# sfu-rsl/FastTrack

Hardware: AMD Instinct MI355X
Metric: frames/sec extract+match (higher is better)
Workload: dtype u8

## Files before the change

### fasttrack_amd/_capi.py

```python
from __future__ import annotations

import ctypes as C
import os
import re

import numpy as np

_PKG = os.path.dirname(os.path.abspath(__file__))
LIB_PATH = os.environ.get("FT_LIB") or os.path.join(_PKG, "libfasttrack_amd.so")
HEADER_PATH = os.path.join(os.path.dirname(_PKG), "include", "fasttrack_amd.h")

FT_OK, FT_ERR_INVALID, FT_ERR_NO_DEVICE, FT_ERR_HIP, FT_ERR_CAPACITY, FT_ERR_EMPTY = 0, -1, -2, -3, -4, -5

KP_DTYPE = np.dtype([("x", "<f4"), ("y", "<f4"), ("size", "<f4"), ("angle", "<f4"), ("response", "<f4"),
                     ("octave", "<i4"), ("class_id", "<i4")])
assert KP_DTYPE.itemsize == 28


class FastTrackError(RuntimeError):
    def __init__(self, status: int, message: str):
        super().__init__(f"fasttrack_amd status {status}: {message}")
        self.status = status


# ... 194 lines not shown
    L.ft_tracked_frame_search_keyframe_projection.argtypes = [vp, C.POINTER(KeyFramePoints), C.POINTER(SE3), f, f, i, i, vp, ip]
    L.ft_tracked_batch_create.argtypes = [vp, i, i, i, C.POINTER(vp)]
    L.ft_tracked_batch_destroy.argtypes = [vp]
    L.ft_tracked_batch_upload.argtypes = [vp, i, C.POINTER(FrameView)]
    L.ft_tracked_batch_search_last_frame.argtypes = [vp, i, C.POINTER(LastPoints), vp, f, vp, vp, i, C.POINTER(vp), vp]
    L.ft_tracked_batch_search_last_frame_se3.argtypes = [vp, i, C.POINTER(LastPoints), C.POINTER(SE3), C.POINTER(SE3), f, vp, vp, i,
                                                         C.POINTER(vp), vp]
    L.ft_tracked_batch_track_local_map.argtypes = [vp, i, C.POINTER(FramePose), C.POINTER(MapPoints), f, f, f, f, i, f,
                                                   C.POINTER(FrustumResult), vp, C.POINTER(vp), vp]
    L.ft_tracked_batch_submit_search_last_frame.argtypes = L.ft_tracked_batch_search_last_frame.argtypes
    L.ft_tracked_batch_submit_search_last_frame_se3.argtypes = L.ft_tracked_batch_search_last_frame_se3.argtypes
    L.ft_tracked_batch_submit_track_local_map.argtypes = L.ft_tracked_batch_track_local_map.argtypes
    L.ft_tracked_batch_wait.argtypes = [vp]
    L.ft_tracked_batch_holder_obs.argtypes = [vp, i, vp]
    L.ft_tracked_batch_bind_fisheye.argtypes = [vp, vp, vp, i, i, i, i, i, i, C.POINTER(FrameView), C.POINTER(FisheyeRig), vp, C.POINTER(vp),
                                                C.POINTER(vp), C.POINTER(vp), C.POINTER(vp), vp]
    L.ft_tracked_batch_bind_fisheye_slots.argtypes = [vp, vp, vp, i, i, i, i, i, i, i, C.POINTER(FrameView), C.POINTER(FisheyeRig), vp,
                                                      C.POINTER(vp), C.POINTER(vp), C.POINTER(vp), C.POINTER(vp), vp]
    L.ft_descriptor_distance.argtypes = [vp, vp, vp, i, vp]
    L.ft_stereo_frontend_device_descriptors.argtypes = [vp, i, i, C.POINTER(vp), ip]
    L.ft_vocabulary_create.argtypes = [vp, i, i, i, i, i, vp, vp, vp, vp, C.POINTER(vp)]
    L.ft_vocabulary_load_text.argtypes = [vp, C.c_char_p, C.POINTER(vp)]
    L.ft_vocabulary_destroy.argtypes = [vp]
    L.ft_vocabulary_info.argtypes = [vp, ip, ip, ip, ip]
    L.ft_bow_transform.argtypes = [vp, vp, i, i, i, vp, vp, vp, vp, vp, i, ip, vp, vp, vp, i, ip]
    L.ft_search_by_bow.argtypes = [vp, C.POINTER(BowSide), vp, C.POINTER(BowSide), i, f, i, vp, ip]
    L.ft_search_for_triangulation.argtypes = [vp, C.POINTER(TriangKeyFrame), i, C.POINTER(TriangKeyFrame), C.POINTER(TriangPair), i, i, i, vp, vp, vp]
    L.ft_fuse_search.argtypes = [vp, C.POINTER(FusePoints), i, C.POINTER(FuseTarget), vp, vp, vp, vp]
    L.ft_search_keyframe_sim3.argtypes = [vp, C.POINTER(FrameView), i, C.POINTER(Sim3Job)]
    L.ft_selftest_libm.argtypes = [vp, i, C.c_uint32, C.c_uint32, C.c_uint32, C.POINTER(C.c_ulonglong),
                                   C.POINTER(C.c_ulonglong), C.POINTER(C.c_uint32)]
    L.ft_octree_distribute.argtypes = [vp, i, i, i, i, i, i, vp, i, ip]
    L.ft_level_geometry.argtypes = [i, i, i, f, i, vp, vp, vp, vp, vp, vp, vp]
    _lib = L
    return L


def check(status: int) -> None:
    if status != FT_OK:
        raise FastTrackError(status, lib().ft_last_error().decode(errors="replace"))


def ptr(a):
    return None if a is None else a.ctypes.data_as(C.c_void_p)
```

### fasttrack_amd/csrc/extractor.cpp

```cpp
#include <algorithm>
#include <map>
#include <cmath>
#include <cstdio>
#include <cstdlib>
#include <cstring>

#include "ft_host.h"

namespace {

inline int cvRoundF(float v) { return (int)lrintf(v); }
inline short satShort(int v) { return (short)(v < -32768 ? -32768 : (v > 32767 ? 32767 : v)); }

#define FT_REQUIRE(cond, msg)                      \
    do {                                           \
        if (!(cond)) {                             \
            ft_set_error(std::string(msg));        \
            return FT_ERR_INVALID;                 \
        }                                          \
    } while (0)

void buildTaps(int ssize, int dsize, bool clampIndex, FtTap *out) {
    const double inv_scale = (double)dsize / ssize;
    const double scale = 1. / inv_scale;
// ... 72 lines not shown
        v.cellBase = cellBase;
        v.cellCap = ((v.wCell + 1) / 2) * ((v.hCell + 1) / 2);
        FT_REQUIRE(v.cellCap < 65536 && v.wCell + 6 < 256 && v.hCell + 6 < 256, "FAST cell too large for the cell records");
        g.fastLv[l] = (unsigned)v.pitch | ((unsigned)v.cellCap << 16);
        v.stageBase = stageBase;
        v.candBase = candBase;
        v.candCap = nCols * nRows * v.cellCap;
        cellBase += nCols * nRows;
        stageBase += v.candCap;
        candBase += v.candCap;
        if (l >= 1) {
            const FtLevelGeom &p = g.lv[l - 1];
            v.area2x = (p.w == 2 * v.w && p.h == 2 * v.h) ? 1 : 0;
            v.xtab = tapOff;
            tapOff += v.w;
            v.ytab = tapOff;
            tapOff += v.h;
        }
        ex->levelMax[l] = ft::octree_max_result(minB, v.maxBX, minB, v.maxBY, ex->quota[l]);
        maxKp += ex->levelMax[l];
    }
    g.totalCells = cellBase;
    g.stagePerSlot = stageBase;
    g.candPerSlot = candBase;
    g.pyrPerSlot = pyrOff;
    g.maxKp = maxKp;
    taps.assign(std::max(tapOff, 1), FtTap{0, 0, 0, 0});
    for (int l = 1; l < L; l++) {
        buildTaps(g.lv[l - 1].w, g.lv[l].w, true, &taps[g.lv[l].xtab]);
        buildTaps(g.lv[l - 1].h, g.lv[l].h, false, &taps[g.lv[l].ytab]);
    }
    return FT_OK;
}

template <typename T>
int devAlloc(T **p, size_t n) {
    FT_HIP(hipMalloc((void **)p, std::max<size_t>(n, 1) * sizeof(T)));
    return FT_OK;
}
template <typename T>
int pinAlloc(T **p, size_t n, unsigned flags = hipHostMallocDefault) {
    FT_HIP(hipHostMalloc((void **)p, std::max<size_t>(n, 1) * sizeof(T), flags));
    return FT_OK;
}

void freeAll(ft_extractor *ex) {
    hipSetDevice(ex->ctx->device);
    if (ex->stream) hipStreamSynchronize(ex->stream);
    if (ex->streamB) hipStreamSynchronize(ex->streamB);
    for (int i = 0; i < FT_OCT_STREAMS; i++)
        if (ex->streamO[i]) hipStreamSynchronize(ex->streamO[i]);
    if (ex->octLayout.prof) {
        unsigned long long h[FT_MAX_LEVELS * 8];
        if (hipMemcpy(h, ex->octLayout.prof, sizeof h, hipMemcpyDeviceToHost) == hipSuccess)
            for (int l = 0; l < ex->nlevels; l++)
                fprintf(stderr, "[oct profile] level %d: codes %.1f us  sort %.1f us  rounds %.1f us (std::sort replay %.1f us, %llu elems in %llu sorts)  pick %.1f us\n",
                        l, h[l * 8] * 0.01, h[l * 8 + 1] * 0.01, h[l * 8 + 2] * 0.01, h[l * 8 + 4] * 0.01, h[l * 8 + 5], h[l * 8 + 6], h[l * 8 + 3] * 0.01);
        hipFree(ex->octLayout.prof);
        ex->octLayout.prof = nullptr;
    }
    ex->evt.destroy();
    for (int i = 0; i < FT_PIPE_MAX; i++) {
        if (ex->evA[i]) hipEventDestroy(ex->evA[i]);
        if (ex->evB[i]) hipEventDestroy(ex->evB[i]);
        if (ex->evO[i]) hipEventDestroy(ex->evO[i]);
    }
// ... 170 lines not shown
            ex->h_srcTab[b].ptr = images[b];
            ex->h_srcTab[b].stride = stride;
            continue;
        }
        uint8_t *stg = ex->h_stage + (size_t)b * width * height;
        for (int y = 0; y < height; y++) memcpy(stg + (size_t)y * width, images[b] + (size_t)y * stride, width);
        ex->h_srcTab[b].ptr = stg;
        ex->h_srcTab[b].stride = width;
    }
}

int ft_extract_ensure_host_cand(ft_extractor *ex) {
    if (ex->h_cand) return FT_OK;
    const size_t n = std::max<size_t>((size_t)ex->maxBatch * ex->geom.candPerSlot, 1);
    FT_HIP(hipHostMalloc((void **)&ex->h_cand, n * sizeof(uint32_t), hipHostMallocMapped | hipHostMallocCoherent));
    void *dp = nullptr;
    FT_HIP(hipHostGetDevicePointer(&dp, ex->h_cand, 0));
    ex->d_cand = (uint32_t *)dp;
    return FT_OK;
}

int ft_extract_launch_a(ft_extractor *ex, int b0, int nb, hipEvent_t done) {
    const FtGeom &g = ex->geom;
    if (!ex->deviceOctree) {
        const int rce = ft_extract_ensure_host_cand(ex);
        if (rce != FT_OK) return rce;
    }
    const bool tm = ex->ctx->kernelTiming;
    const int al = ex->l0Aligned ? 1 : 0;
    const uint8_t *const *l0 = ex->d_l0 + b0;
    uint8_t *pyr = ex->d_pyr + (size_t)b0 * g.pyrPerSlot;
    int *cellCount = ex->d_cellCount + (size_t)b0 * g.totalCells;
    uint32_t *stage = ex->d_stage + (size_t)b0 * g.stagePerSlot;
    ex->evt.begin(tm, "kernel.pyr_down(all levels)", ex->stream);
    int rc = ft_launch_pyramid(ex->stream, g, nb, l0, ex->l0pitch, pyr, ex->d_taps, al, ex->tune.pyr_rows);
    ex->evt.end(tm, ex->stream);
    if (rc != FT_OK) return rc;
    ex->evt.begin(tm, "kernel.fast_cells", ex->stream);
    rc = ft_launch_fast_cells(ex->stream, g, nb, l0, ex->l0pitch, pyr, ex->iniTh, ex->minTh, al, cellCount, stage,
                              ex->deviceOctree ? 0 : 1, ex->d_cellTab);
    ex->evt.end(tm, ex->stream);
    if (rc != FT_OK) return rc;
    ex->evt.begin(tm, "kernel.compact", ex->stream);
    uint32_t *candDst = ex->deviceOctree ? ex->d_candDev : ex->d_cand;
    int *cntDst = ex->deviceOctree ? ex->d_candCountDev : ex->d_candCount;
    rc = ft_launch_compact(ex->stream, g, nb, cellCount, stage, candDst + (size_t)b0 * g.candPerSlot,
                           cntDst + (size_t)b0 * g.nlevels);
    ex->evt.end(tm, ex->stream);
    if (rc != FT_OK) return rc;
    if (done) FT_HIP(hipEventRecord(done, ex->stream));
    return FT_OK;
}

int ft_extract_launch_octree(ft_extractor *ex, int sub, int b0, int nb, hipEvent_t done) {
    const FtGeom &g = ex->geom;
    hipStream_t so = ex->streamO[sub % FT_OCT_STREAMS];
    FT_HIP(hipEventRecord(ex->evO[sub], ex->stream));
    FT_HIP(hipStreamWaitEvent(so, ex->evO[sub], 0));
    FtOctArgs a = ex->octLayout;
    a.cand = ex->d_candDev + (size_t)b0 * g.candPerSlot;
    a.candCount = ex->d_candCountDev + (size_t)b0 * g.nlevels;
    a.sel = ex->d_sel + (size_t)b0 * g.maxKp;
    a.selCount = ex->d_selCount + (size_t)b0 * g.nlevels;
    a.overflow = ex->d_overflow;
    a.ovSlot = ex->d_ovSlot + b0;
    a.low = ex->d_octLow ? ex->d_octLow + (size_t)b0 * g.nlevels * FT_OCT_MAXN : nullptr;
    const bool large = nb > 16 || ex->lastBatch > 16;
    const bool histNow = ex->histEnabled && (large ? ex->histGrid > 0 : ex->histOn);
// ... 273 lines not shown
int ft_extractor_create(ft_context *ctx, int nfeatures, float scale_factor, int nlevels, int ini_th_fast,
                        int min_th_fast, int image_width, int image_height, int max_batch, ft_extractor **out) {
    FT_REQUIRE(ctx && out, "ft_extractor_create: null argument");
    *out = nullptr;
    FT_REQUIRE(nfeatures > 0, "nfeatures must be positive");
    FT_REQUIRE(nlevels >= 1 && nlevels <= FT_MAX_LEVELS, "nlevels outside [1, 12]");
    FT_REQUIRE(scale_factor > 1.0f, "scaleFactor must exceed 1");
    FT_REQUIRE(min_th_fast >= 1 && ini_th_fast >= min_th_fast && ini_th_fast < 255,
               "FAST thresholds must satisfy 1 <= minThFAST <= iniThFAST < 255");
    FT_REQUIRE(image_width >= 2 * FT_EDGE_THRESHOLD + 8 && image_height >= 2 * FT_EDGE_THRESHOLD + 8,
               "image smaller than the 19-px border allows");
    FT_REQUIRE(max_batch >= 1 && max_batch <= 4096, "max_batch outside [1, 4096]");
    int rc = ft_set_device(ctx);
    if (rc != FT_OK) return rc;
    ft_extractor *ex = new ft_extractor();
    ex->ctx = ctx;
    ex->nfeatures = nfeatures;
    ex->scaleFactor = scale_factor;
    ex->nlevels = nlevels;
    ex->iniTh = ini_th_fast;
    ex->minTh = min_th_fast;
    ex->width = image_width;
    ex->height = image_height;
    ex->maxBatch = max_batch;
    ex->tune = ctx->tuning;
    std::vector<FtTap> taps;
    rc = buildGeometry(ex, taps);
    if (rc != FT_OK) {
        delete ex;
        return rc;
    }
    const FtGeom &g = ex->geom;
    const size_t B = max_batch;
#define FT_TRY(x)            \
    do {                     \
        rc = (x);            \
        if (rc != FT_OK) {   \
            freeAll(ex);     \
            delete ex;       \
            return rc;       \
        }                    \
    } while (0)
    {
        hipStream_t lanes[FT_LANE_STREAMS];
        FT_TRY(ft_context_take_lanes(ctx, max_batch <= 16, image_width, image_height, lanes, &ex->ownStreams));
        ex->stream = lanes[0];
        ex->streamB = lanes[1];
        for (int i = 0; i < FT_OCT_STREAMS; i++) ex->streamO[i] = lanes[2 + i];
    }
    hipError_t se = hipSuccess;
    for (int i = 0; i < FT_PIPE_MAX && se == hipSuccess; i++) {
        se = hipEventCreateWithFlags(&ex->evA[i], hipEventDisableTiming);
        if (se == hipSuccess) se = hipEventCreateWithFlags(&ex->evB[i], hipEventDisableTiming);
        if (se == hipSuccess) se = hipEventCreateWithFlags(&ex->evO[i], hipEventDisableTiming);
        if (se == hipSuccess && i == 0) se = hipEventCreateWithFlags(&ex->evJoin, hipEventDisableTiming);
        if (se == hipSuccess && i == 0) se = hipEventCreateWithFlags(&ex->evUp, hipEventDisableTiming);
    }
    if (se != hipSuccess) {
        freeAll(ex);
        delete ex;
        return ft_hip_fail(se, "stream / event creation", __FILE__, __LINE__);
    }
    FT_TRY(devAlloc(&ex->d_pyr, B * g.pyrPerSlot));
    FT_TRY(devAlloc(&ex->d_taps, taps.size()));
    FT_TRY(devAlloc(&ex->d_cellTab, (size_t)std::max(g.totalCells, 1)));
    FT_TRY(devAlloc(&ex->d_cellCount, B * g.totalCells));
// ... 148 lines not shown
        return FT_ERR_CAPACITY;
    }
    *n_out = k;
    if (k > capacity) {
        ft_set_error("ft_octree_distribute: capacity too small");
        return FT_ERR_CAPACITY;
    }
    for (int i = 0; i < k; i++) out_idx[i] = keep[i];
    return FT_OK;
}

int ft_level_geometry(int width, int height, int nfeatures, float scale_factor, int nlevels, int *level_w,
                      int *level_h, int *quota, int *n_cols, int *n_rows, int *w_cell, int *h_cell) {
    FT_REQUIRE(nlevels >= 1 && nlevels <= FT_MAX_LEVELS && scale_factor > 1.0f && nfeatures > 0, "bad parameters");
    ft_extractor ex;
    ex.nfeatures = nfeatures;
    ex.scaleFactor = scale_factor;
    ex.nlevels = nlevels;
    ex.width = width;
    ex.height = height;
    std::vector<FtTap> taps;
    int rc = buildGeometry(&ex, taps);
    if (rc != FT_OK) return rc;
    for (int l = 0; l < nlevels; l++) {
        const FtLevelGeom &v = ex.geom.lv[l];
        if (level_w) level_w[l] = v.w;
        if (level_h) level_h[l] = v.h;
        if (quota) quota[l] = ex.quota[l];
        if (n_cols) n_cols[l] = v.nCols;
        if (n_rows) n_rows[l] = v.nRows;
        if (w_cell) w_cell[l] = v.wCell;
        if (h_cell) h_cell[l] = v.hCell;
    }
    return FT_OK;
}

int ft_extractor_destroy(ft_extractor *ex) {
    if (!ex) return FT_OK;
    freeAll(ex);
    ex->ctx->liveObjects--;
    delete ex;
    return FT_OK;
}

int ft_extractor_levels(const ft_extractor *ex) { return ex ? ex->nlevels : 0; }
int ft_extractor_max_batch(const ft_extractor *ex) { return ex ? ex->maxBatch : 0; }
int ft_extractor_max_keypoints(const ft_extractor *ex) { return ex ? ex->geom.maxKp : 0; }

int ft_extractor_scale_factors(const ft_extractor *ex, float *scale, float *inv_scale, float *sigma2,
                               float *inv_sigma2) {
    FT_REQUIRE(ex, "null extractor");
    for (int i = 0; i < ex->nlevels; i++) {
        if (scale) scale[i] = ex->sf[i];
        if (inv_scale) inv_scale[i] = ex->invsf[i];
        if (sigma2) sigma2[i] = ex->sigma2[i];
        if (inv_sigma2) inv_sigma2[i] = ex->invsigma2[i];
    }
    return FT_OK;
}

int ft_extractor_features_per_level(const ft_extractor *ex, int *quota) {
    FT_REQUIRE(ex && quota, "null argument");
    for (int i = 0; i < ex->nlevels; i++) quota[i] = ex->quota[i];
    return FT_OK;
}

// ... 411 lines not shown
```

### fasttrack_amd/csrc/ft_host.h

```cpp
#pragma once

#include <atomic>
#include <chrono>
#include <map>
#include <mutex>
#include <string>
#include <vector>

#include "ft_internal.h"
#include "octree.h"
#include "thread_pool.h"

#define FT_PIPE_MAX 8
#define FT_LANE_SMALL_PIXELS ((size_t)600 * 1000)
#define FT_LANE_MAP_SMALL {1, 2, 3, 4, 2, 1, 3, 1, 5, 4, 3, 2, 1, 1, 0, 1}
#define FT_OCT_STREAMS 2
#define FT_LANE_STREAMS (2 + FT_OCT_STREAMS)

#define FT_TUNING_OPTIONS(X)                                                                                                  \
    X(pipeline_depth, "FT_PIPELINE_DEPTH", 0, 0, 8, "sub-batches a throughput batch is enqueued as (0 = automatic, 1 = no pipelining, <= 8)") \
    X(device_octree, "FT_DEVICE_OCTREE", 1, 0, 1, "DistributeOctTree on the device (0 = host thread pool)")                  \
    X(oct_hist, "FT_OCT_HIST", 1, 0, 1, "histogram tier of the device octree for levels above 4096 candidates")              \
    X(oct_hist_first, "FT_OCT_HIST_FIRST", 1, 0, 2, "histogram formulation for every level: 0 never, 1 latency-mode launches, 2 always") \
    X(oct_big, "FT_OCT_BIG", 1, 0, 1, "sorted big tier of the device octree (up to 16384 keys per level)")                   \
    X(pyr_rows, "FT_PYR_ROWS", 1, 0, 1, "pyramid of launches of 8+ images: 1 = row-streaming kernel (k_pyr_rows), 0 = tile kernel (k_pyr_down)") \
    X(upload_kernel, "FT_UPLOAD_KERNEL", 1, 0, 1, "latency mode: frames go up through k_upload instead of DMA copies")       \
    X(graph, "FT_GRAPH", 1, 0, 1, "latency mode: batches of <= 8 frames are captured and replayed as HIP graphs")            \
    X(paired, "FT_PAIRED", 1, 0, 1, "latency-mode stereo front ends run both cameras through one set of launches")           \
    X(pass_burst, "FT_PASS_BURST", 12, 2, 14, "projection searches: claim passes enqueued per host round trip")              \
    X(search_cache, "FT_SEARCH_CACHE", 2, 0, 3, "projection searches: 1 = later claim passes walk the cached candidate keys, 2 = and a batch of 24+ frames resolves its claims in one launch, 3 = every batch does") \
    X(search_grid, "FT_SEARCH_GRID", 1, 0, 1, "projection searches: CSR grid of the frame built on the device") \
    X(blocking_sync, "FT_BLOCKING_SYNC", 2, 0, 2, "host waits for the device: 0 = the runtime's default (it spins), 1 = sleeping (hipDeviceScheduleBlockingSync), 2 = sleeping when the process may use fewer than 8 CPUs")

struct ft_tuning {
#define FT_X(field, env, def, lo, hi, doc) int field = def;
    FT_TUNING_OPTIONS(FT_X)
#undef FT_X
};
bool ft_tuning_from_env(ft_tuning &t, std::string &err);
int *ft_tuning_field(ft_tuning &t, const char *name);
const char *ft_debug_env(const char *name);
const char *ft_read_env(const char *name);

struct ft_context {
    int device = 0;
    std::string deviceName;
    ft::ThreadPool *pool = nullptr;
    hipStream_t stream = nullptr;
    std::mutex laneMutex;
    std::vector<hipStream_t> lanes;
    hipStream_t uploadStream = nullptr;
    std::vector<int> laneMap;
    std::vector<int> laneMapSmall;
    bool userLaneMap = false;
    int nextLaneSet = 0;
    size_t maxPitch = 0;
    int hwQueues = 4;
    std::atomic<int> liveObjects{0};
// ... 44 lines not shown
        hipEventRecord(recs.back().b, st);
    }
    void resolve(ft_context *ctx) {
        for (auto &r : recs) {
            float ms = 0;
            if (hipEventElapsedTime(&ms, r.a, r.b) == hipSuccess) ctx->addStat(r.name, ms);
        }
        recs.clear();
        used = 0;
    }
    void destroy() {
        for (auto e : pool) hipEventDestroy(e);
        pool.clear();
    }
};

struct FtTimer {
    std::chrono::steady_clock::time_point t0 = std::chrono::steady_clock::now();
    double ms() const {
        return std::chrono::duration<double, std::milli>(std::chrono::steady_clock::now() - t0).count();
    }
};

struct ft_extractor {
    ft_context *ctx = nullptr;
    ft_tuning tune;
    int nfeatures = 0, nlevels = 0, iniTh = 0, minTh = 0, width = 0, height = 0, maxBatch = 0;
    float scaleFactor = 1.2f;
    std::vector<float> sf, invsf, sigma2, invsigma2;
    std::vector<int> quota;
    std::vector<int> levelMax;
    std::vector<int> levelOff;
    FtGeom geom{};
    hipStream_t stream = nullptr;
    hipStream_t streamB = nullptr;
    hipEvent_t evA[FT_PIPE_MAX] = {}, evB[FT_PIPE_MAX] = {};
    hipStream_t streamO[FT_OCT_STREAMS] = {};
    bool ownStreams = false;
    hipEvent_t evO[FT_PIPE_MAX] = {};
    struct GraphKey {
        int batch = 0, onDevice = 0, width = 0, height = 0, stride = 0, aligned = 0, bigGrid = 0;
        bool operator==(const GraphKey &o) const {
            return batch == o.batch && onDevice == o.onDevice && width == o.width && height == o.height && stride == o.stride &&
                   aligned == o.aligned && bigGrid == o.bigGrid;
        }
    } graphKey;
    hipGraphExec_t graphExec = nullptr;
    bool graphDisabled = false;
    hipEvent_t evJoin = nullptr;
    hipEvent_t evUp = nullptr;
    hipEvent_t foreignReader = nullptr;
    uint8_t *d_pyr = nullptr;
    FtTap *d_taps = nullptr;
    FtCellRec *d_cellTab = nullptr;
    int *d_cellCount = nullptr;
    uint32_t *d_stage = nullptr;
    const uint8_t **d_l0 = nullptr;
    const uint8_t **h_l0 = nullptr;
    uint8_t *h_stage = nullptr;
    FtSrcEntry *h_srcTab = nullptr;
    bool stageHost = false;
    float *d_sf = nullptr;
    uint32_t *h_cand = nullptr, *d_cand = nullptr;
    int *h_candCount = nullptr, *d_candCount = nullptr;
    bool deviceOctree = false;
    uint32_t *d_candDev = nullptr;
// ... 109 lines not shown
```

### fasttrack_amd/csrc/ft_internal.h

```cpp
#pragma once

#include <hip/hip_runtime.h>
#include <stdint.h>

#include <string>

#include "../../include/fasttrack_amd.h"

#define FT_MAX_LEVELS 12
#define FT_EDGE_THRESHOLD 19
#define FT_PATCH_SIZE 31
#define FT_HALF_PATCH 15
#define FT_TH_HIGH 100
#define FT_TH_LOW 50
#define FT_HISTO_LENGTH 30
#define FT_GRID_COLS 64
#define FT_GRID_ROWS 48

struct FtLevelGeom {
    int w, h, pitch;
    int off;
    int maxBX, maxBY;
    int nCols, nRows, wCell, hCell;
    int cellBase;
// ... 94 lines not shown
};

struct FtBowTree {
    const int *childStart;
    const unsigned *childList;
    const uint8_t *desc;
    const unsigned *wordId;
    const double *weight;
    int nNodes;
};
int ft_launch_bow_walk(hipStream_t st, const FtBowTree &t, const uint8_t *desc, int n, int nidLevel, unsigned *wordOut,
                       unsigned *nodeOut, double *weightOut);
struct FtBowSide {
    int n, nNodes;
    const unsigned *nodes;
    const int *offsets;
    const unsigned *features;
    const uint8_t *desc;
};
int ft_launch_search_by_bow(hipStream_t st, const FtBowSide &K, const uint8_t *kfHasPoint, const FtBowSide &F, int nleft,
                            float nnRatio, int *matches);

void ft_set_error(const std::string &msg);
int ft_debug_repeat(const char *name);
int ft_hip_fail(hipError_t e, const char *what, const char *file, int line);
const char *ft_debug_env(const char *name);

#define FT_HIP(call)                                                              \
    do {                                                                          \
        hipError_t _e = (call);                                                   \
        if (_e != hipSuccess) return ft_hip_fail(_e, #call, __FILE__, __LINE__);  \
    } while (0)

int ft_launch_pyramid(hipStream_t st, const FtGeom &g, int batch, const uint8_t *const *l0, int l0pitch,
                      uint8_t *pyr, const FtTap *taps, int alignedLoads, int rowsKernel);
struct FtCellRanges {
    int lo0, n0, lo1, n1;
};
int ft_launch_fast_cells(hipStream_t st, const FtGeom &g, int batch, const uint8_t *const *l0, int l0pitch,
                         const uint8_t *pyr, int iniTh, int minTh, int alignedLoads, int *cellCount,
                         uint32_t *stage, int ordered, const FtCellRec *cellTab);
int ft_launch_compact(hipStream_t st, const FtGeom &g, int batch, const int *cellCount, const uint32_t *stage,
                      uint32_t *cand, int *candCount);
int ft_launch_orient_desc(hipStream_t st, const FtGeom &g, int batch, const uint8_t *const *l0, int l0pitch,
                          const uint8_t *pyr, int alignedLoads, const FtSelKp *sel, const int *selCount,
                          const FtOctArgs &layout, int *nSel, ft_keypoint *keys, uint8_t *desc);
int ft_launch_octree(hipStream_t st, const FtGeom &g, int batch, const FtOctArgs &a);
int ft_launch_blur_level(hipStream_t st, const uint8_t *img, int pitch, int w, int h, uint8_t *dst, int dstPitch);
size_t ft_octree_smem_bytes(int poolCap, bool compact = false);
size_t ft_octree_hist_smem_bytes(int poolCap);
int ft_octree_big_keys(int poolCap);
size_t ft_fast_smem_bytes(const FtGeom &g);

struct __attribute__((aligned(16))) FtSortedR {
    float x, y;
    int octave, idx;
    unsigned long long desc[4];
};
struct FtStereoArgs {
    const ft_keypoint *keysL, *keysR;
    const uint8_t *descL, *descR;
    const int *nL, *nR;
    int capacity;
    float mbf, mb;
    float *uright, *depth;
    int *sad;
    int *hamIdx;
    int *nMatches;
// ... 62 lines not shown
```

### fasttrack_amd/csrc/kernels_extract.hip

```cpp
#include "ft_internal.h"
#include "libm_f32.h"
#include "wave_ops.h"

namespace {


struct FtMomentTab {
    unsigned W[17 * 8], M[17 * 8];
};
constexpr FtMomentTab ft_make_moment_tab() {
    constexpr int umax[16] = {15, 15, 15, 15, 14, 14, 14, 13, 13, 12, 11, 10, 9, 8, 6, 3};
    FtMomentTab t{};
    for (int av = 0; av < 16; av++)
        for (int j = 0; j < 8; j++)
            for (int k = 0; k < 4; k++) {
                const int u = -15 + 4 * j + k;
                const int au = u < 0 ? -u : u;
                if (u <= 15 && au <= umax[av]) {
                    t.W[av * 8 + j] |= (unsigned)(u + 16) << (8 * k);
                    t.M[av * 8 + j] |= 1u << (8 * k);
                }
            }
    return t;
}
// ... 153 lines not shown
    for (int j = 0; j < 4; j++) {
        const int dy = by + j;
        if (dy > dy1) break;
        const int sy0 = min(max((int)yt[j].s, 0), sh - 1) - sya, sy1 = min(max((int)yt[j].s + 1, 0), sh - 1) - sya;
        const uint8_t *r0 = T + __mul24(sy0, ldsPitch), *r1 = T + __mul24(sy1, ldsPitch);
        unsigned pk = 0;
#pragma unroll
        for (int k = 0; k < 4; k++) {
            const int h0 = r0[cx0[k]] * xt[k].a0 + r0[cx1[k]] * xt[k].a1;
            const int h1 = r1[cx0[k]] * xt[k].a0 + r1[cx1[k]] * xt[k].a1;
            pk |= (unsigned)(((vmul24((int)yt[j].a0, h0 >> 4) >> 16) + (vmul24((int)yt[j].a1, h1 >> 4) >> 16) + 2) >> 2) << (8 * k);
        }
        gstore<unsigned>(outLevel + (unsigned)vmad24(dy, D.pitch, bx), pk);
    }
}

#define PR_COLS 128
#ifndef PR_RB
#define PR_RB 32
#endif
#ifndef PR_PF
#define PR_PF 4
#endif
typedef unsigned short ft_us2 __attribute__((ext_vector_type(2)));
typedef unsigned ft_u2 __attribute__((ext_vector_type(2)));
__device__ __forceinline__ unsigned udot2_u16(unsigned a, unsigned b) {
    return __builtin_amdgcn_udot2(__builtin_bit_cast(ft_us2, a), __builtin_bit_cast(ft_us2, b), 0u, false);
}
__device__ __forceinline__ unsigned umulhi_su(unsigned bShifted16, unsigned a) {
    unsigned r;
    asm("v_mul_hi_u32 %0, %1, %2" : "=v"(r) : "s"(bShifted16), "v"(a));
    return r;
}
template <bool AREA>
__global__ __launch_bounds__(64) void k_pyr_rows(FtGeom g, int level, const uint8_t *const *l0, int l0pitch, uint8_t *pyr,
                                                 const FtTap *taps, FtSlotGrid sg, int stripsX, unsigned sxMagic,
                                                 int readableEnd) {
    const int lane = threadIdx.x;
    int slot, tile;
    if (!ft_slot_block(sg, slot, tile)) return;
    const int ty = div_by(tile, sxMagic), tx = tile - ty * stripsX;
    const FtLevelGeom &D = g.lv[level];
    int spitch;
    const uint8_t *S = level_ptr(g, level - 1, slot, l0, l0pitch, pyr, spitch);
    const int sw = g.lv[level - 1].w, sh = g.lv[level - 1].h;
    const int dx = tx * PR_COLS + 2 * lane;
    const int j0 = ty * PR_RB, nrows = min(PR_RB, D.h - j0);
    unsigned rowW0 = 0, rowW1 = 0;
    if constexpr (!AREA) {
        const ft_u2 t = gload<ft_u2>(taps + D.ytab + j0 + min(lane, nrows - 1));
        const int sy = (int)(short)(t.x & 0xffffu);
        rowW0 = (unsigned)min(max(sy, 0), sh - 1) | ((unsigned)min(max(sy + 1, 0), sh - 1) << 16);
        rowW1 = (t.x >> 16) | (t.y << 16);
        if (lane >= nrows) rowW0 = 0xffffffffu;
    }
    const int dxa = min(dx, D.w - 1), dxb = min(dx + 1, D.w - 1);
    int sxa, sxb, cxa, cxb;
    unsigned wa, wb;
    if constexpr (AREA) {
        sxa = 2 * dxa; sxb = 2 * dxb; cxa = sxa + 1; cxb = sxb + 1;
        wa = wb = 0x00010001u;
    } else {
        const ft_u2 ta = gload<ft_u2>(taps + D.xtab + dxa), tb = gload<ft_u2>(taps + D.xtab + dxb);
        sxa = (int)(short)(ta.x & 0xffffu); sxb = (int)(short)(tb.x & 0xffffu);
        cxa = min(sxa + 1, sw - 1); cxb = min(sxb + 1, sw - 1);
        wa = (ta.x >> 16) | (ta.y << 16);
        wb = (tb.x >> 16) | (tb.y << 16);
    }
    const int base = min(sxa & ~3, readableEnd - 8);
    const unsigned selA = (unsigned)(sxa - base) | 0x0c00u | ((unsigned)(cxa - base) << 16) | 0x0c000000u;
    const unsigned selB = (unsigned)(sxb - base) | 0x0c00u | ((unsigned)(cxb - base) << 16) | 0x0c000000u;
    auto rowTap = [&](int r, int &sy0, int &sy1, unsigned &b0, unsigned &b1) {
        if constexpr (AREA) {
            sy0 = 2 * (j0 + r); sy1 = r < nrows ? sy0 + 1 : -1; b0 = b1 = 0;
        } else {
            const unsigned w0 = (unsigned)__builtin_amdgcn_readlane((int)rowW0, r), w1 = (unsigned)__builtin_amdgcn_readlane((int)rowW1, r);
            sy0 = (int)(w0 & 0xffffu); sy1 = (int)(w0 >> 16);
            b0 = w1 << 16; b1 = w1 & 0xffff0000u;
        }
    };
// ... 37 lines not shown
                    asm volatile("" : "+v"(hpA), "+v"(hpB));
                }
                unsigned oA, oB;
                if constexpr (AREA) {
                    oA = (hpA + hcA + 2u) >> 2; oB = (hpB + hcB + 2u) >> 2;
                } else {
                    oA = (umulhi_su(b0, hpA) + umulhi_su(b1, hcA) + 2u) >> 2;
                    oB = (umulhi_su(b0, hpB) + umulhi_su(b1, hcB) + 2u) >> 2;
                }
                unsigned offD = laneDst + dOff;
                asm volatile("" : "+v"(offD));
                if constexpr (!EDGE) {
                    gstore<unsigned short>(dstBase + offD, (unsigned short)(oA | (oB << 8)));
                } else {
                    if (store2) gstore<unsigned short>(dstBase + offD, (unsigned short)(oA | (oB << 8)));
                    else if (store1) gstore<uint8_t>(dstBase + offD, (uint8_t)oA);
                }
                dOff += (unsigned)D.pitch;
                jr++;
                rowTap(jr, sy0, sy1, b0, b1);
            }
            r++;
        };
        for (int left = rLast - r + 1; left > 0; left -= PR_PF) {
#pragma unroll
            for (int k = 0; k < PR_PF; k++) {
                take(q[k]);
                step();
            }
        }
    };
    if (tx * PR_COLS + PR_COLS <= D.w) run(std::false_type{});
    else run(std::true_type{});
}

typedef unsigned short fs_us2 __attribute__((ext_vector_type(2)));
__device__ __forceinline__ unsigned pk_max_u16(unsigned a, unsigned b) {
    return __builtin_bit_cast(unsigned, __builtin_elementwise_max(__builtin_bit_cast(fs_us2, a), __builtin_bit_cast(fs_us2, b)));
}
__device__ __forceinline__ unsigned pk_min_u16(unsigned a, unsigned b) {
    return __builtin_bit_cast(unsigned, __builtin_elementwise_min(__builtin_bit_cast(fs_us2, a), __builtin_bit_cast(fs_us2, b)));
}
__device__ __forceinline__ bool has_arc9(unsigned m) {
    unsigned d = m | (m << 16);
    unsigned a = d & (d >> 1);
    a &= a >> 2;
    a &= a >> 4;
    a &= d >> 8;
    return (a & 0xffffu) != 0;
}

#define FT_RING(F)                                                                                            \
    F(0, 0, 3) F(1, 1, 3) F(2, 2, 2) F(3, 3, 1) F(4, 3, 0) F(5, 3, -1) F(6, 2, -2) F(7, 1, -3) F(8, 0, -3)    \
    F(9, -1, -3) F(10, -2, -2) F(11, -3, -1) F(12, -3, 0) F(13, -3, 1) F(14, -2, 2) F(15, -1, 3)

__device__ __forceinline__ int fast_score(int v, const int p[16]) {
    int mn3[16], mx3[16];
#pragma unroll
    for (int k = 0; k < 16; k++) {
        mn3[k] = min(min(p[k], p[(k + 1) & 15]), p[(k + 2) & 15]);
        mx3[k] = max(max(p[k], p[(k + 1) & 15]), p[(k + 2) & 15]);
    }
    int mn9[16], mx9[16];
#pragma unroll
    for (int k = 0; k < 16; k++) {
        mn9[k] = min(min(mn3[k], mn3[(k + 3) & 15]), mn3[(k + 6) & 15]);
// ... 964 lines not shown
        }
    }
    if (profW && lane == 0) atomicAdd(&g_odProf[0], 1ull);
}

}

static int fast_tile_pitch(const FtGeom &g) {
    int need = 0;
    for (int l = 0; l < g.nlevels; l++)
        if (g.lv[l].nCols * g.lv[l].nRows > 0) need = std::max(need, g.lv[l].wCell + 9);
    return need <= 48 ? 48 : (need <= 64 ? 64 : 0);
}

size_t ft_fast_smem_bytes(const FtGeom &g) {
    const int TP = fast_tile_pitch(g);
    size_t mxTile = 0, mxScore = 0, mxSum = 0;
    for (int l = 0; l < g.nlevels; l++) {
        const FtLevelGeom &L = g.lv[l];
        const size_t t = (size_t)fc_tile_bytes(L.wCell, L.hCell, TP), sc = (size_t)fc_score_bytes(L.wCell, L.hCell, TP);
        mxTile = std::max(mxTile, t);
        mxScore = std::max(mxScore, sc);
        mxSum = std::max(mxSum, t + sc);
    }
    return (TP ? mxTile + mxScore : mxSum) + fc_list_bytes();
}

static bool pyr_rows_fits(const FtGeom &g, int level) {
    const FtLevelGeom &D = g.lv[level], &P = g.lv[level - 1];
    return (double)P.w / (double)D.w < 2.5 && P.w >= 8;
}

int ft_launch_pyramid(hipStream_t st, const FtGeom &g, int batch, const uint8_t *const *l0, int l0pitch,
                      uint8_t *pyr, const FtTap *taps, int alignedLoads, int rowsKernel) {
    const bool rowsOn = rowsKernel != 0;
    for (int rep = ft_debug_repeat("pyr"); rep > 0; rep--)
    for (int level = 1; level < g.nlevels; level++) {
        const FtLevelGeom &D = g.lv[level], &P = g.lv[level - 1];
        if (rowsOn && batch >= 8 && alignedLoads && pyr_rows_fits(g, level)) {
            const int stripsX = (D.w + PR_COLS - 1) / PR_COLS, stripsY = (D.h + PR_RB - 1) / PR_RB;
            dim3 grid, block(64, 1, 1);
            const FtSlotGrid sg = ft_slot_grid(stripsX * stripsY, batch, grid);
            const int readableEnd = level == 1 ? std::min((P.w + 3) & ~3, l0pitch) : P.pitch;
            if (D.area2x)
                hipLaunchKernelGGL(k_pyr_rows<true>, grid, block, 0, st, g, level, l0, l0pitch, pyr, taps, sg, stripsX,
                                   div_magic_of((unsigned)stripsX), readableEnd);
            else
                hipLaunchKernelGGL(k_pyr_rows<false>, grid, block, 0, st, g, level, l0, l0pitch, pyr, taps, sg, stripsX,
                                   div_magic_of((unsigned)stripsX), readableEnd);
            continue;
        }
        const int cols = (int)((long long)PD_TW * P.w / D.w) + 8, rowsN = (int)((long long)PD_TH * P.h / D.h) + 8;
        const int ldsPitch = (cols + 3 + 3) & ~3;
        const unsigned sxQ16 = (unsigned)(((unsigned long long)P.w << 16) / (unsigned)D.w) + 1u;
        const unsigned syQ16 = (unsigned)(((unsigned long long)P.h << 16) / (unsigned)D.h) + 1u;
        const int tilesX = (D.w + PD_TW - 1) / PD_TW, tilesY = (D.h + PD_TH - 1) / PD_TH;
        dim3 grid, block(64, 1, 1);
        const FtSlotGrid sg = ft_slot_grid(tilesX * tilesY, batch, grid);
        hipLaunchKernelGGL(k_pyr_down, grid, block, (size_t)ldsPitch * rowsN + 4, st, g, level, l0, l0pitch, pyr, taps,
                           alignedLoads, ldsPitch, rowsN, sxQ16, syQ16, sg, tilesX, div_magic_of((unsigned)tilesX));
    }
    FT_HIP(hipGetLastError());
    return FT_OK;
}

static size_t fast_smem_of(const FtGeom &g, unsigned mask, int TP, int *tileBytes, int *scoreBytes) {
    size_t mxTile = 0, mxScore = 0, mxSum = 0;
    for (int l = 0; l < g.nlevels; l++) {
// ... 155 lines not shown
```

### include/fasttrack_amd.h

```cpp
#ifndef FASTTRACK_AMD_H
#define FASTTRACK_AMD_H

#include <stddef.h>
#include <stdint.h>

#ifdef __cplusplus
extern "C" {
#endif

#define FT_API __attribute__((visibility("default")))

typedef enum ft_status {
    FT_OK = 0,
    FT_ERR_INVALID = -1,
    FT_ERR_NO_DEVICE = -2,
    FT_ERR_HIP = -3,
    FT_ERR_CAPACITY = -4,
    FT_ERR_EMPTY = -5
} ft_status;

typedef struct ft_keypoint {
    float x, y, size, angle, response;
    int octave, class_id;
} ft_keypoint;
// ... 32 lines not shown
                               int min_th_fast, int image_width, int image_height, int max_batch,
                               ft_extractor **out);
FT_API int ft_extractor_destroy(ft_extractor *ex);
FT_API int ft_extractor_levels(const ft_extractor *ex);
FT_API int ft_extractor_max_batch(const ft_extractor *ex);
FT_API int ft_extractor_max_keypoints(const ft_extractor *ex);
FT_API int ft_extractor_scale_factors(const ft_extractor *ex, float *scale, float *inv_scale, float *sigma2,
                                      float *inv_sigma2);
FT_API int ft_extractor_features_per_level(const ft_extractor *ex, int *quota);
FT_API int ft_extractor_level_size(const ft_extractor *ex, int level, int *width, int *height);

FT_API int ft_extract(ft_extractor *ex, const uint8_t *image, int width, int height, int stride, int lap0,
                      int lap1, ft_keypoint *keypoints, uint8_t *descriptors, int capacity, int *n_keypoints,
                      int *n_mono);


FT_API int ft_extract_batch(ft_extractor *ex, const uint8_t *const *images, int batch, int on_device, int width,
                            int height, int stride, int lap0, int lap1, ft_keypoint *keypoints,
                            uint8_t *descriptors, int capacity, int *n_keypoints, int *n_mono);

FT_API int ft_extractor_download_level(ft_extractor *ex, int slot, int level, uint8_t *dst, int dst_stride);
FT_API int ft_extractor_download_blurred_level(ft_extractor *ex, int slot, int level, uint8_t *dst, int dst_stride);
FT_API int ft_extractor_device_level(ft_extractor *ex, int slot, int level, const uint8_t **dptr, int *pitch);
FT_API int ft_extractor_download_candidates(ft_extractor *ex, int slot, int level, int *xys, int capacity,
                                            int *n);

FT_API int ft_extractor_octree_on_device(ft_extractor *ex, int level, const int *xys, int n, int tiers, int *out_xys,
                                         int capacity, int *n_out, int *tier);

FT_API int ft_octree_distribute(const int *xys, int n, int minX, int maxX, int minY, int maxY, int N, int *out_idx,
                                int capacity, int *n_out);
FT_API int ft_level_geometry(int width, int height, int nfeatures, float scale_factor, int nlevels, int *level_w,
                             int *level_h, int *quota, int *n_cols, int *n_rows, int *w_cell, int *h_cell);

FT_API int ft_stereo_match(ft_extractor *exL, ft_extractor *exR, int slot, const ft_keypoint *keysL, int nL,
                           const ft_keypoint *keysR, int nR, const uint8_t *descL, const uint8_t *descR,
                           float mbf, float mb, int apply_median_cut, float *uright, float *depth, int *sad,
                           int *n_matches);

typedef struct ft_stereo_frontend ft_stereo_frontend;
FT_API int ft_stereo_frontend_create(ft_context *ctx, int nfeatures, float scale_factor, int nlevels,
                                     int ini_th_fast, int min_th_fast, int image_width, int image_height,
                                     int max_batch, float mbf, float mb, ft_stereo_frontend **out);
FT_API int ft_stereo_frontend_destroy(ft_stereo_frontend *fe);
FT_API ft_extractor *ft_stereo_frontend_left(ft_stereo_frontend *fe);
FT_API ft_extractor *ft_stereo_frontend_right(ft_stereo_frontend *fe);
FT_API int ft_stereo_frontend_submit(ft_stereo_frontend *fe, const uint8_t *const *imagesL,
                                     const uint8_t *const *imagesR, int batch, int on_device, int width, int height,
                                     int stride, ft_keypoint *keysL, uint8_t *descL, int *nL, ft_keypoint *keysR,
                                     uint8_t *descR, int *nR, int capacity, float *uright, float *depth,
                                     int *n_matches);
FT_API int ft_stereo_frontend_wait(ft_stereo_frontend *fe);
FT_API int ft_stereo_frontend_process(ft_stereo_frontend *fe, const uint8_t *const *imagesL,
                                      const uint8_t *const *imagesR, int batch, int on_device, int width,
                                      int height, int stride, ft_keypoint *keysL, uint8_t *descL, int *nL,
                                      ft_keypoint *keysR, uint8_t *descR, int *nR, int capacity, float *uright,
                                      float *depth, int *n_matches);
FT_API int ft_stereo_frontend_device_descriptors(ft_stereo_frontend *fe, int slot, int right, const uint8_t **dptr, int *n);

FT_API int ft_fisheye_match(ft_context *ctx, const uint8_t *descL, int nL, const uint8_t *descR, int nR,
                            int *matches, int *best, int *second);

typedef struct ft_fisheye_rig {
    float cam1[8], cam2[8];
    float precision;
    float Rlr[9], tlr[3];
// ... 283 lines not shown
```

Baseline: 79730.

## Fuse all pyramid levels into one cascade launch with per-band workgroups

Adds k_pyr_cascade, which builds every pyramid level in a single launch. Each workgroup of 16 waves owns a horizontal band of one image, with band row ranges precomputed on the host and widened so each band holds all source rows the next level needs. Workgroup barriers separate the levels, so the per-level launch count and the inter-launch gaps go away. In exchange, each level's parallelism is capped at batch×bands workgroups, rows overlapping between bands are computed redundantly, and the whole workgroup waits at every level barrier. It becomes the default for launches of 8+ images and is skipped during graph capture.

```diff
diff --git a/fasttrack_amd/_capi.py b/fasttrack_amd/_capi.py
--- a/fasttrack_amd/_capi.py
+++ b/fasttrack_amd/_capi.py
@@ -250,6 +250,7 @@
                                    C.POINTER(C.c_ulonglong), C.POINTER(C.c_uint32)]
     L.ft_octree_distribute.argtypes = [vp, i, i, i, i, i, i, vp, i, ip]
     L.ft_level_geometry.argtypes = [i, i, i, f, i, vp, vp, vp, vp, vp, vp, vp]
+    L.ft_pyramid_band_plan.argtypes = [i, i, f, i, i, vp, vp]
     _lib = L
     return L
 
diff --git a/fasttrack_amd/csrc/extractor.cpp b/fasttrack_amd/csrc/extractor.cpp
--- a/fasttrack_amd/csrc/extractor.cpp
+++ b/fasttrack_amd/csrc/extractor.cpp
@@ -128,6 +128,43 @@
     }
     return FT_OK;
 }
+
+}
+
+void ft_pyr_bands_of(const FtGeom &g, int K, int *first, int *end) {
+    for (int k = 0; k < K; k++) first[k] = end[k] = 0;
+    std::vector<FtTap> yt;
+    for (int k = 0; k < K; k++) {
+        int lo = 0, hi = 0;
+        for (int l = g.nlevels - 1; l >= 1; l--) {
+            const int H = g.lv[l].h;
+            int a = (int)((long long)k * H / K), b = (int)((long long)(k + 1) * H / K);
+            if (hi > lo) {
+                int s0, s1;
+                if (g.lv[l + 1].area2x) {
+                    s0 = 2 * lo;
+                    s1 = 2 * (hi - 1) + 2;
+                } else {
+                    yt.resize(g.lv[l + 1].h);
+                    buildTaps(H, g.lv[l + 1].h, false, yt.data());
+                    s0 = std::min(std::max((int)yt[lo].s, 0), H - 1);
+                    s1 = std::min(std::max((int)yt[hi - 1].s + 1, 0), H - 1) + 1;
+                }
+                if (b > a) {
+                    a = std::min(a, s0);
+                    b = std::max(b, s1);
+                } else {
+                    a = s0;
+                    b = s1;
+                }
+            }
+            first[l * K + k] = lo = a;
+            end[l * K + k] = hi = b;
+        }
+    }
+}
+
+namespace {
 
 template <typename T>
 int devAlloc(T **p, size_t n) {
@@ -364,8 +401,11 @@
     uint8_t *pyr = ex->d_pyr + (size_t)b0 * g.pyrPerSlot;
     int *cellCount = ex->d_cellCount + (size_t)b0 * g.totalCells;
     uint32_t *stage = ex->d_stage + (size_t)b0 * g.stagePerSlot;
+    hipStreamCaptureStatus cap = hipStreamCaptureStatusNone;
+    FT_HIP(hipStreamIsCapturing(ex->stream, &cap));
     ex->evt.begin(tm, "kernel.pyr_down(all levels)", ex->stream);
-    int rc = ft_launch_pyramid(ex->stream, g, nb, l0, ex->l0pitch, pyr, ex->d_taps, al, ex->tune.pyr_rows);
+    int rc = ft_launch_pyramid(ex->stream, g, nb, l0, ex->l0pitch, pyr, ex->d_taps, al, ex->tune.pyr_rows,
+                               cap == hipStreamCaptureStatusNone ? &ex->pyrBands : nullptr);
     ex->evt.end(tm, ex->stream);
     if (rc != FT_OK) return rc;
     ex->evt.begin(tm, "kernel.fast_cells", ex->stream);
@@ -705,6 +745,13 @@
     }
     const FtGeom &g = ex->geom;
     const size_t B = max_batch;
+    {
+        int first[FT_MAX_LEVELS * PC_BANDS], end[FT_MAX_LEVELS * PC_BANDS];
+        ft_pyr_bands_of(g, PC_BANDS, first, end);
+        ex->pyrBands.K = PC_BANDS;
+        for (int l = 1; l < g.nlevels; l++)
+            for (int k = 0; k < PC_BANDS; k++) ex->pyrBands.rows[l][k] = (unsigned)first[l * PC_BANDS + k] | ((unsigned)end[l * PC_BANDS + k] << 16);
+    }
 #define FT_TRY(x)            \
     do {                     \
         rc = (x);            \
@@ -919,6 +966,21 @@
         if (w_cell) w_cell[l] = v.wCell;
         if (h_cell) h_cell[l] = v.hCell;
     }
+    return FT_OK;
+}
+
+int ft_pyramid_band_plan(int width, int height, float scale_factor, int nlevels, int bands, int *first_row, int *end_row) {
+    FT_REQUIRE(nlevels >= 1 && nlevels <= FT_MAX_LEVELS && scale_factor > 1.0f && bands >= 1 && first_row && end_row, "bad parameters");
+    ft_extractor ex;
+    ex.nfeatures = 1000;
+    ex.scaleFactor = scale_factor;
+    ex.nlevels = nlevels;
+    ex.width = width;
+    ex.height = height;
+    std::vector<FtTap> taps;
+    int rc = buildGeometry(&ex, taps);
+    if (rc != FT_OK) return rc;
+    ft_pyr_bands_of(ex.geom, bands, first_row, end_row);
     return FT_OK;
 }
 
diff --git a/fasttrack_amd/csrc/ft_host.h b/fasttrack_amd/csrc/ft_host.h
--- a/fasttrack_amd/csrc/ft_host.h
+++ b/fasttrack_amd/csrc/ft_host.h
@@ -23,7 +23,7 @@
     X(oct_hist, "FT_OCT_HIST", 1, 0, 1, "histogram tier of the device octree for levels above 4096 candidates")              \
     X(oct_hist_first, "FT_OCT_HIST_FIRST", 1, 0, 2, "histogram formulation for every level: 0 never, 1 latency-mode launches, 2 always") \
     X(oct_big, "FT_OCT_BIG", 1, 0, 1, "sorted big tier of the device octree (up to 16384 keys per level)")                   \
-    X(pyr_rows, "FT_PYR_ROWS", 1, 0, 1, "pyramid of launches of 8+ images: 1 = row-streaming kernel (k_pyr_rows), 0 = tile kernel (k_pyr_down)") \
+    X(pyr_rows, "FT_PYR_ROWS", 2, 0, 2, "pyramid of launches of 8+ images: 2 = all levels in one launch, a workgroup per band of an image (k_pyr_cascade), 1 = row-streaming kernel, a launch per level (k_pyr_rows), 0 = tile kernel (k_pyr_down)") \
     X(upload_kernel, "FT_UPLOAD_KERNEL", 1, 0, 1, "latency mode: frames go up through k_upload instead of DMA copies")       \
     X(graph, "FT_GRAPH", 1, 0, 1, "latency mode: batches of <= 8 frames are captured and replayed as HIP graphs")            \
     X(paired, "FT_PAIRED", 1, 0, 1, "latency-mode stereo front ends run both cameras through one set of launches")           \
@@ -134,6 +134,7 @@
     std::vector<int> levelMax;
     std::vector<int> levelOff;
     FtGeom geom{};
+    FtPyrBands pyrBands{};
     hipStream_t stream = nullptr;
     hipStream_t streamB = nullptr;
     hipEvent_t evA[FT_PIPE_MAX] = {}, evB[FT_PIPE_MAX] = {};
diff --git a/fasttrack_amd/csrc/ft_internal.h b/fasttrack_amd/csrc/ft_internal.h
--- a/fasttrack_amd/csrc/ft_internal.h
+++ b/fasttrack_amd/csrc/ft_internal.h
@@ -150,8 +150,20 @@
         if (_e != hipSuccess) return ft_hip_fail(_e, #call, __FILE__, __LINE__);  \
     } while (0)
 
+#ifndef PC_BANDS
+#define PC_BANDS 2
+#endif
+#ifndef PC_WAVES
+#define PC_WAVES 16
+#endif
+#define FT_PYR_BANDS_MAX 8
+struct FtPyrBands {
+    int K;
+    unsigned rows[FT_MAX_LEVELS][FT_PYR_BANDS_MAX];
+};
+void ft_pyr_bands_of(const FtGeom &g, int K, int *first, int *end);
 int ft_launch_pyramid(hipStream_t st, const FtGeom &g, int batch, const uint8_t *const *l0, int l0pitch,
-                      uint8_t *pyr, const FtTap *taps, int alignedLoads, int rowsKernel);
+                      uint8_t *pyr, const FtTap *taps, int alignedLoads, int rowsKernel, const FtPyrBands *bands);
 struct FtCellRanges {
     int lo0, n0, lo1, n1;
 };
diff --git a/fasttrack_amd/csrc/kernels_extract.hip b/fasttrack_amd/csrc/kernels_extract.hip
--- a/fasttrack_amd/csrc/kernels_extract.hip
+++ b/fasttrack_amd/csrc/kernels_extract.hip
@@ -209,20 +209,13 @@
     asm("v_mul_hi_u32 %0, %1, %2" : "=v"(r) : "s"(bShifted16), "v"(a));
     return r;
 }
-template <bool AREA>
-__global__ __launch_bounds__(64) void k_pyr_rows(FtGeom g, int level, const uint8_t *const *l0, int l0pitch, uint8_t *pyr,
-                                                 const FtTap *taps, FtSlotGrid sg, int stripsX, unsigned sxMagic,
-                                                 int readableEnd) {
-    const int lane = threadIdx.x;
-    int slot, tile;
-    if (!ft_slot_block(sg, slot, tile)) return;
-    const int ty = div_by(tile, sxMagic), tx = tile - ty * stripsX;
+template <bool AREA, bool BAND>
+__device__ __forceinline__ void pyr_rows_strip(const FtGeom &g, int level, int slot, int tx, int j0, int rowEnd, int lane,
+                                               const uint8_t *S, int spitch, uint8_t *pyr, const FtTap *taps, int readableEnd) {
     const FtLevelGeom &D = g.lv[level];
-    int spitch;
-    const uint8_t *S = level_ptr(g, level - 1, slot, l0, l0pitch, pyr, spitch);
     const int sw = g.lv[level - 1].w, sh = g.lv[level - 1].h;
     const int dx = tx * PR_COLS + 2 * lane;
-    const int j0 = ty * PR_RB, nrows = min(PR_RB, D.h - j0);
+    const int nrows = min(PR_RB, (BAND ? rowEnd : D.h) - j0);
     unsigned rowW0 = 0, rowW1 = 0;
     if constexpr (!AREA) {
         const ft_u2 t = gload<ft_u2>(taps + D.ytab + j0 + min(lane, nrows - 1));
@@ -326,6 +319,49 @@
     };
     if (tx * PR_COLS + PR_COLS <= D.w) run(std::false_type{});
     else run(std::true_type{});
+}
+
+template <bool AREA>
+__global__ __launch_bounds__(64) void k_pyr_rows(FtGeom g, int level, const uint8_t *const *l0, int l0pitch, uint8_t *pyr,
+                                                 const FtTap *taps, FtSlotGrid sg, int stripsX, unsigned sxMagic,
+                                                 int readableEnd) {
+    const int lane = threadIdx.x;
+    int slot, tile;
+    if (!ft_slot_block(sg, slot, tile)) return;
+    const int ty = div_by(tile, sxMagic), tx = tile - ty * stripsX;
+    int spitch;
+    const uint8_t *S = level_ptr(g, level - 1, slot, l0, l0pitch, pyr, spitch);
+    pyr_rows_strip<AREA, false>(g, level, slot, tx, ty * PR_RB, 0, lane, S, spitch, pyr, taps, readableEnd);
+}
+
+__global__ __launch_bounds__(64 * PC_WAVES) void k_pyr_cascade(FtGeom g, const uint8_t *const *l0, int l0pitch, uint8_t *pyr,
+                                                              const FtTap *taps, FtSlotGrid sg, FtPyrBands pb,
+                                                              int l0ReadableEnd) {
+    const int lane = threadIdx.x & 63, wave = wave_index();
+    int slot, band;
+    if (!ft_slot_block(sg, slot, band)) return;
+    const uint8_t *const frame = l0[slot];
+    for (int level = 1; level < g.nlevels; level++) {
+        const unsigned rr = pb.rows[level][band];
+        const int r0 = (int)(rr & 0xffffu), r1 = (int)(rr >> 16);
+        const int stripsX = (g.lv[level].w + PR_COLS - 1) / PR_COLS;
+        const unsigned sxMagic = div_magic_small((unsigned)stripsX);
+        const int n = stripsX * ((r1 - r0 + PR_RB - 1) / PR_RB);
+        const int readableEnd = level == 1 ? l0ReadableEnd : g.lv[level - 1].pitch;
+        const int spitch = level == 1 ? l0pitch : g.lv[level - 1].pitch;
+        const uint8_t *S = level == 1 ? frame : pyr + (size_t)slot * g.pyrPerSlot + g.lv[level - 1].off;
+        for (int s = wave; s < n; s += PC_WAVES) {
+            const int ty = div_by(s, sxMagic), tx = s - ty * stripsX;
+            const int j0 = r0 + ty * PR_RB;
+            if (g.lv[level].area2x) pyr_rows_strip<true, true>(g, level, slot, tx, j0, r1, lane, S, spitch, pyr, taps, readableEnd);
+            else pyr_rows_strip<false, true>(g, level, slot, tx, j0, r1, lane, S, spitch, pyr, taps, readableEnd);
+        }
+        if (level + 1 < g.nlevels) {
+            __builtin_amdgcn_fence(__ATOMIC_RELEASE, "workgroup");
+            __syncthreads();
+            __builtin_amdgcn_fence(__ATOMIC_ACQUIRE, "workgroup");
+        }
+    }
 }
 
 typedef unsigned short fs_us2 __attribute__((ext_vector_type(2)));
@@ -1356,8 +1392,19 @@
 }
 
 int ft_launch_pyramid(hipStream_t st, const FtGeom &g, int batch, const uint8_t *const *l0, int l0pitch,
-                      uint8_t *pyr, const FtTap *taps, int alignedLoads, int rowsKernel) {
+                      uint8_t *pyr, const FtTap *taps, int alignedLoads, int rowsKernel, const FtPyrBands *bands) {
     const bool rowsOn = rowsKernel != 0;
+    bool cascade = rowsKernel == 2 && batch >= 8 && alignedLoads && bands && bands->K >= 1 && g.nlevels >= 2;
+    for (int level = 1; cascade && level < g.nlevels; level++) cascade = pyr_rows_fits(g, level);
+    if (cascade) {
+        dim3 grid, block(64 * PC_WAVES, 1, 1);
+        const FtSlotGrid sg = ft_slot_grid(bands->K, batch, grid);
+        const int readableEnd = std::min((g.lv[0].w + 3) & ~3, l0pitch);
+        for (int rep = ft_debug_repeat("pyr"); rep > 0; rep--)
+            hipLaunchKernelGGL(k_pyr_cascade, grid, block, 0, st, g, l0, l0pitch, pyr, taps, sg, *bands, readableEnd);
+        FT_HIP(hipGetLastError());
+        return FT_OK;
+    }
     for (int rep = ft_debug_repeat("pyr"); rep > 0; rep--)
     for (int level = 1; level < g.nlevels; level++) {
         const FtLevelGeom &D = g.lv[level], &P = g.lv[level - 1];
diff --git a/include/fasttrack_amd.h b/include/fasttrack_amd.h
--- a/include/fasttrack_amd.h
+++ b/include/fasttrack_amd.h
@@ -88,6 +88,7 @@
                                 int capacity, int *n_out);
 FT_API int ft_level_geometry(int width, int height, int nfeatures, float scale_factor, int nlevels, int *level_w,
                              int *level_h, int *quota, int *n_cols, int *n_rows, int *w_cell, int *h_cell);
+FT_API int ft_pyramid_band_plan(int width, int height, float scale_factor, int nlevels, int bands, int *first_row, int *end_row);
 
 FT_API int ft_stereo_match(ft_extractor *exL, ft_extractor *exR, int slot, const ft_keypoint *keysL, int nL,
                            const ft_keypoint *keysR, int nR, const uint8_t *descL, const uint8_t *descR,
```

After: 83660, median of 6. +4.9%, better.
